# jaswon/osu-dreamer

Hardware: AMD Instinct MI355X
Metric: denoiser train-steps/sec + 50-step sample latents/sec, 1/2/4/8 MI355X (higher is better)
Workload: dtype bf16

## Files before the change

include/osu_dreamer_hip.h:

```cpp
#ifndef OSU_DREAMER_HIP_H
#define OSU_DREAMER_HIP_H

#ifdef __cplusplus
extern "C" {
#endif

enum { OD_F32 = 0, OD_BF16 = 1,
       OD_F32X3 = 2,
       OD_F32X3W = 3,
       OD_F16 = 4 };
enum { OD_EPI_NONE = 0, OD_EPI_SILU = 1 };
enum { OD_ACT_NONE = 0, OD_ACT_SILU = 1 };
enum { OD_ERR_ARG = -1, OD_ERR_ALIGN = -2, OD_ERR_UNSUPPORTED = -3, OD_ERR_COMM = -4 };

int od_version(void);
const char* od_build_source_sha(void);
const char* od_error_string(int code);

int od_gemm_nt(int dtype, const void* A, int lda, const void* W, int ldw, const float* bias, void* C, int ldc,
               int M, int N, int K, int epilogue, int accumulate, void* stream);
int od_gemm_nt_qkrope(int dtype, const void* A, int lda, const void* W, int ldw, const float* bias, void* C, int ldc, int M,
                      int N, int K, const float* wq, const float* wk, const float* table, int L, int H, int hd, float eps,
                      float q_scale, void* stream);
int od_gemm_nt_qkrope_split(int dtype, const void* A, int lda, const void* W, int ldw, const float* bias, void* C, int ldc,
// ... 15 lines not shown
int od_cl_to_frames(int dtype, const float* src, void* dst, int ldd, int B, int C, int L, void* stream);
int od_proj_in(int dtype, const float* xt, const float* W, const float* bias, void* x, int ldx, int B, int E, int L,
               int D, void* stream);
int od_proj_in_bwd(int dtype, const float* xt, const void* dx, int ldx, float* dW, float* db, int B, int E, int L, int D,
                   void* stream);
int od_silu(int dtype, const void* x, void* y, long n, void* stream);
int od_silu_bwd(int dtype, const void* x, const void* dy, void* dx, long n, void* stream);

int od_rmsnorm_film(int dtype, const void* x, int ldx, const float* ssg, const void* cl, int ldcl, int cl_bcast,
                    void* h, int ldh, float* inv_rms, int B, int L, int C, float eps, void* stream);
int od_rmsnorm_film_bwd(int dtype, const void* x, int ldx, const float* inv_rms, const float* ssg, const void* dh,
                        int lddh, void* dres, int lddres, float* dssg, int B, int L, int C, void* stream);
int od_rmsnorm_gate_residual(int dtype, const void* x, int ldx, const void* h, int ldh, const float* ssg, void* xo,
                             int ldxo, float* inv_rms, int B, int L, int C, float eps, void* stream);
int od_rmsnorm_gate_residual_film(int dtype, const void* x, int ldx, const void* h, int ldh, const float* ssg_a, void* xo, int ldxo,
                                  float* inv_a, const float* ssg_b, const void* cl, int ldcl, int cl_bcast, void* h2, int ldh2,
                                  float* inv_b, int B, int L, int C, float eps, void* stream);
int od_rmsnorm_gate_residual_film_dwconv(int dtype, const void* x, int ldx, const void* h, int ldh, const float* ssg_a, void* xo, int ldxo,
                                         float* inv_a, const float* ssg_b, void* h2, int ldh2, float* inv_b, const float* conv_w,
                                         const float* conv_b, void* y, int ldy, int B, int L, int C, int ksize, float eps, void* stream);
int od_rmsnorm_gate_residual_bwd(int dtype, const void* h, int ldh, const float* inv_rms, const float* ssg,
                                 const void* dy, int lddy, void* dh, int lddh, float* dssg, int B, int L, int C,
                                 void* stream);

int od_rope_table(float* table, int L, int hd, void* stream);
int od_qk_norm_rope(int dtype, const void* qkv, int ldqkv, const float* wq, const float* wk, const float* table,
                    void* qk_out, int ldo, int B, int L, int H, int hd, float eps, float q_scale, void* stream);
int od_qk_norm_rope_bwd(int dtype, const void* qkv, int ldqkv, const float* wq, const float* wk, const float* table,
                        const void* dqk, int lddqk, void* dqkv, int lddqkv, float* dwq, float* dwk, int B, int L,
                        int H, int hd, float eps, float q_scale, void* stream);
int od_flash_attn_fwd(int dtype, const void* q, int ldq, const void* k, int ldk, const void* v, int ldv, void* o, int ldo,
                      float* lse, int B, int H, int L, int hd, float scale, int q_prescaled, void* stream);
int od_flash_attn_fwd_varlen(int dtype, const void* q, int ldq, const void* k, int ldk, const void* v, int ldv, void* o, int ldo,
                             float* lse, const int* lens, int B, int H, int L, int hd, float scale, int q_prescaled, void* stream);
int od_flash_attn_bwd(int dtype, const void* q, int ldq, const void* k, int ldk, const void* v, int ldv, const void* o,
                      int ldo, const void* dout, int lddo, const float* lse, float* delta, void* dq, int lddq, void* dk,
                      int lddk, void* dv, int lddv, int B, int H, int L, int hd, float scale, int q_prescaled, void* stream);
int od_attn_aux_create(void** aux_out);
int od_attn_aux_destroy(void* aux);
int od_flash_attn_bwd_aux(int dtype, const void* q, int ldq, const void* k, int ldk, const void* v, int ldv, const void* o,
                          int ldo, const void* dout, int lddo, const float* lse, float* delta, void* dq, int lddq, void* dk,
                          int lddk, void* dv, int lddv, int B, int H, int L, int hd, float scale, int q_prescaled, void* aux, void* stream);
int od_flash_attn_bwd_fused_ws_bytes(int dtype, int B, int H, int L, long* total_out, long* zero_out);
int od_flash_attn_bwd_fused(int dtype, const void* q, int ldq, const void* k, int ldk, const void* v, int ldv, const void* o, int ldo,
                            const void* dout, int lddo, const float* lse, void* dq, int lddq, void* dk, int lddk, void* dv, int lddv,
                            int B, int H, int L, int hd, float scale, int q_prescaled, void* ws, long ws_bytes, void* stream);
// ... 129 lines not shown
```

osu_dreamer_amd/csrc/heads.hip:

```cpp
#include "od_common.h"
#include "od_api_internal.h"

namespace {

constexpr int UW = 32;
constexpr int UOWN = 30;
constexpr int UWPB = 4;
constexpr int MAXU = 64, MAXE = 8;

__device__ __forceinline__ float red32(float v) {
#pragma unroll
    for (int m = 16; m >= 1; m >>= 1) v += __shfl_xor(v, m);
    return v;
}

struct UHeadW {
    const float *w0, *b0, *w1, *b1, *w3, *b3, *w4, *b4;
};

struct UHeadSmem {
    float xts[MAXE][UW + 4];
    float z0s[MAXE][UW + 2];
    float z1s[MAXU][UW + 2];
    float a1s[MAXU][UW + 2];
// ... 17 lines not shown
    }
    __syncthreads();
    for (int idx = t; idx < U * (UW + 2); idx += 256) {
        const int c = idx / (UW + 2), i2 = idx % (UW + 2);
        const int f = l0 - 2 + i2;
        float z = P.b1[c];
        for (int e = 0; e < E; e++) z += P.w1[c * E + e] * S.z0s[e][i2];
        S.z1s[c][i2] = z;
        S.a1s[c][i2] = (f >= 0 && f < Lv) ? od_silu(z) : 0.f;
    }
    __syncthreads();
    for (int idx = t; idx < U * UW; idx += 256) {
        const int c = idx / UW, i = idx % UW;
        S.z3s[c][i] = P.b3[c] + P.w3[c * 3 + 0] * S.a1s[c][i] + P.w3[c * 3 + 1] * S.a1s[c][i + 1] + P.w3[c * 3 + 2] * S.a1s[c][i + 2];
    }
    __syncthreads();
}

__device__ __forceinline__ void uhead_load_w4(UHeadSmem& S, const UHeadW& P, int U) {
    for (int idx = threadIdx.x; idx < U * U; idx += 256) S.w4s[idx / U][idx % U] = P.w4[idx];
    __syncthreads();
}

template <bool VL = false>
__global__ __launch_bounds__(256) void uhead_fwd_kernel(const float* __restrict__ xt, UHeadW P, float* __restrict__ fsum,
                                                        int E, int L, int U, int nwin, int wpb, const OdDetTable* __restrict__ det,
                                                        const int* __restrict__ lens = nullptr) {
    __shared__ UHeadSmem S;
    const int b = blockIdx.y, t = threadIdx.x;
    const int Lb = VL ? od_uniform(lens[b]) : L;
    const int i = t & 31, grp = t >> 5, cpg = U / 8;
    uhead_load_w4(S, P, U);
    float acc[MAXU / 8];
#pragma unroll
    for (int q = 0; q < MAXU / 8; q++) acc[q] = 0.f;
    for (int wi = 0; wi < wpb; wi++) {
        const int win = blockIdx.x * wpb + wi;
        if (win >= nwin) break;
        const int l0 = win * UOWN;
        if (VL && l0 >= Lb) break;
        uhead_window_fwd(S, xt, P, b, l0, E, L, U, Lb);
        const int f = l0 - 1 + i;
        const bool own = (i >= 1 && i < UW - 1 && f < Lb);
#pragma unroll
        for (int q = 0; q < MAXU / 8; q++) {
            if (q < cpg) {
                const int c = grp * cpg + q;
                float z = P.b4[c];
                for (int cc = 0; cc < U; cc++) z += S.w4s[c][cc] * S.z3s[cc][i];
                if (own) acc[q] += od_silu(z);
            }
        }
        __syncthreads();
    }
#pragma unroll
    for (int q = 0; q < MAXU / 8; q++) {
        const float s = red32(acc[q]);
        if (q < cpg && i == 0) od_red_add(det, fsum + (size_t)b * U + grp * cpg + q, s);
    }
}

struct UHeadG {
    float *dw0, *db0, *dw1, *db1, *dw3, *db3, *dw4, *db4;
};

__global__ __launch_bounds__(256) void uhead_bwd_kernel(const float* __restrict__ xt, UHeadW P, const float* __restrict__ dfm,
                                                        UHeadG G, int E, int L, int U, int nwin, const OdDetTable* __restrict__ det) {
    __shared__ UHeadSmem S;
    __shared__ float sdw3[MAXU][3], sdb3[MAXU], sdb4[MAXU], sdw1[MAXU][MAXE], sdb1[MAXU], sdw0[MAXE][3], sdb0[MAXE];
    const int b = blockIdx.y, t = threadIdx.x;
    const int i = t & 31, grp = t >> 5, cpg = U / 8;
    for (int idx = t; idx < MAXU; idx += 256) {
        sdb3[idx] = 0.f; sdb4[idx] = 0.f; sdb1[idx] = 0.f;
        for (int j = 0; j < 3; j++) sdw3[idx][j] = 0.f;
        for (int e = 0; e < MAXE; e++) sdw1[idx][e] = 0.f;
    }
    if (t < MAXE) { sdb0[t] = 0.f; for (int j = 0; j < 3; j++) sdw0[t][j] = 0.f; }
    uhead_load_w4(S, P, U);
    float adw4[16];
#pragma unroll
    for (int q = 0; q < 16; q++) adw4[q] = 0.f;
    const float invL = 1.0f / (float)L;

    for (int wi = 0; wi < UWPB; wi++) {
        const int win = blockIdx.x * UWPB + wi;
        if (win >= nwin) break;
        const int l0 = win * UOWN;
        uhead_window_fwd(S, xt, P, b, l0, E, L, U, L);
        const int f = l0 - 1 + i;
        const bool inr = (f >= 0 && f < L);
        const bool own = (i >= 1 && i < UW - 1 && f < L);
#pragma unroll
        for (int q = 0; q < MAXU / 8; q++) {
            if (q < cpg) {
                const int c = grp * cpg + q;
                float z = P.b4[c];
                for (int cc = 0; cc < U; cc++) z += S.w4s[c][cc] * S.z3s[cc][i];
                const float g = inr ? dfm[(size_t)b * U + c] * invL * od_silu_grad(z) : 0.f;
                S.g4s[c][i] = g;
                const float s = red32(own ? g : 0.f);
                if (i == 0) atomicAdd(&sdb4[c], s);
            }
        }
        __syncthreads();
        {
            const int iend = (L - (l0 - 1)) < (UW - 1) ? (L - (l0 - 1)) : (UW - 1);
#pragma unroll
            for (int q = 0; q < 16; q++) {
                const int o = t + 256 * q;
                if (o < U * U) {
                    const int c = o / U, cc = o % U;
                    float s = 0.f;
                    for (int ii = 1; ii < iend; ii++) s += S.g4s[c][ii] * S.z3s[cc][ii];
                    adw4[q] += s;
                }
            }
        }
        __syncthreads();
        float dz3v[MAXU / 8];
#pragma unroll
        for (int q = 0; q < MAXU / 8; q++) {
            dz3v[q] = 0.f;
            if (q < cpg) {
                const int cc = grp * cpg + q;
                float s = 0.f;
                for (int c = 0; c < U; c++) s += S.w4s[c][cc] * S.g4s[c][i];
                dz3v[q] = s;
            }
        }
        __syncthreads();
#pragma unroll
        for (int q = 0; q < MAXU / 8; q++)
            if (q < cpg) S.z3s[grp * cpg + q][i] = dz3v[q];
        __syncthreads();
#pragma unroll
        for (int q = 0; q < MAXU / 8; q++) {
            if (q < cpg) {
                const int c = grp * cpg + q;
                const float g = own ? S.z3s[c][i] : 0.f;
                float s = red32(g);
                if (i == 0) atomicAdd(&sdb3[c], s);
                for (int j = 0; j < 3; j++) {
                    s = red32(g * S.a1s[c][i + j]);
                    if (i == 0) atomicAdd(&sdw3[c][j], s);
                }
                float dz1 = 0.f;
                if (own) {
                    float da1 = 0.f;
                    for (int j = 0; j < 3; j++) da1 += P.w3[c * 3 + j] * S.z3s[c][i - j + 1];
                    dz1 = da1 * od_silu_grad(S.z1s[c][i + 1]);
                }
                S.g4s[c][i] = dz1;
                s = red32(dz1);
                if (i == 0) atomicAdd(&sdb1[c], s);
                for (int e = 0; e < E; e++) {
                    s = red32(dz1 * S.z0s[e][i + 1]);
                    if (i == 0) atomicAdd(&sdw1[c][e], s);
                }
            }
        }
        __syncthreads();
        {
            const bool ev = grp < E;
            const int e = ev ? grp : 0;
            float dz0 = 0.f;
            if (ev)
                for (int c = 0; c < U; c++) dz0 += P.w1[c * E + e] * S.g4s[c][i];
            float s = red32(dz0);
            if (ev && i == 0) atomicAdd(&sdb0[e], s);
            for (int j = 0; j < 3; j++) {
                s = red32(dz0 * S.xts[e][i + 1 + j]);
                if (ev && i == 0) atomicAdd(&sdw0[e][j], s);
            }
        }
        __syncthreads();
    }
#pragma unroll
    for (int q = 0; q < 16; q++) {
        const int o = t + 256 * q;
        if (o < U * U) od_red_add(det, G.dw4 + o, adw4[q]);
    }
    __syncthreads();
    for (int c = t; c < U; c += 256) {
        od_red_add(det, G.db4 + c, sdb4[c]);
        od_red_add(det, G.db3 + c, sdb3[c]);
        od_red_add(det, G.db1 + c, sdb1[c]);
        for (int j = 0; j < 3; j++) od_red_add(det, G.dw3 + c * 3 + j, sdw3[c][j]);
        for (int e = 0; e < E; e++) od_red_add(det, G.dw1 + c * E + e, sdw1[c][e]);
    }
    if (t < E) {
        od_red_add(det, G.db0 + t, sdb0[t]);
        for (int j = 0; j < 3; j++) od_red_add(det, G.dw0 + t * 3 + j, sdw0[t][j]);
    }
}

template <bool VL = false>
__global__ void uhead_tail_kernel(const float* __restrict__ fsum, const float* __restrict__ mod, const float* __restrict__ w,
                                  const float* __restrict__ bo, float* __restrict__ u, int B, int U, int L, float u_scale,
                                  const int* __restrict__ lens = nullptr) {
    const int b = blockIdx.x, lane = threadIdx.x;
    const float Lf = (float)(VL ? od_uniform(lens[b]) : L);
    float s = 0.f;
    for (int c = lane; c < U; c += 64) {
        const float f = fsum[(size_t)b * U + c] / Lf;
        s += w[c] * (f * (1.f + mod[(size_t)b * 2 * U + c]) + mod[(size_t)b * 2 * U + U + c]);
    }
    s = od_wave_sum(s);
    if (lane == 0) {
        const float y = s + bo[0];
        const float sp = y > 20.f ? y : log1pf(__expf(y));
        u[b] = u_scale * sp;
    }
}
__global__ void uhead_tail_bwd_kernel(const float* __restrict__ fsum, const float* __restrict__ mod, const float* __restrict__ w,
                                      const float* __restrict__ bo, const float* __restrict__ du, float* __restrict__ dfm,
                                      float* __restrict__ dmod, float* __restrict__ dw, float* __restrict__ dbo,
// ... 158 lines not shown
extern "C" int od_uhead_fwd_varlen(const float* xt, const float* w0, const float* b0, const float* w1, const float* b1, const float* w3,
                                   const float* b3, const float* w4, const float* b4, float* fsum, const int* lens, int B, int E, int L,
                                   int U, void* stream) {
    if (U > MAXU || U % 8 || E > MAXE) return OD_ERR_UNSUPPORTED;
    if (!lens) return OD_ERR_ARG;
    const int nwin = (L + UOWN - 1) / UOWN;
    UHeadW P{w0, b0, w1, b1, w3, b3, w4, b4};
    int wpb = (int)((long)nwin * B / 512);
    wpb = wpb < 1 ? 1 : (wpb > UWPB ? UWPB : wpb);
    OD_LAUNCH(uhead_fwd_kernel<true>, dim3((nwin + wpb - 1) / wpb, B), dim3(256), 0, (hipStream_t)stream, xt, P, fsum, E, L, U, nwin, wpb,
              od_det_active(), lens);
    OD_CHECK_LAUNCH();
    return 0;
}

extern "C" int od_uhead_bwd(const float* xt, const float* w0, const float* b0, const float* w1, const float* b1, const float* w3,
                            const float* b3, const float* w4, const float* b4, const float* dfm, float* dw0, float* db0,
                            float* dw1, float* db1, float* dw3, float* db3, float* dw4, float* db4, int B, int E, int L, int U,
                            void* stream) {
    if (U > MAXU || U % 8 || E > MAXE) return OD_ERR_UNSUPPORTED;
    const int nwin = (L + UOWN - 1) / UOWN;
    UHeadW P{w0, b0, w1, b1, w3, b3, w4, b4};
    UHeadG G{dw0, db0, dw1, db1, dw3, db3, dw4, db4};
    OD_LAUNCH(uhead_bwd_kernel, dim3((nwin + UWPB - 1) / UWPB, B), dim3(256), 0, (hipStream_t)stream, xt, P, dfm, G, E, L, U, nwin, od_det_active());
    OD_CHECK_LAUNCH();
    return 0;
}

extern "C" int od_uhead_tail(const float* fsum, const float* mod, const float* w_out, const float* b_out, float* u, int B, int U,
                             int L, float u_scale, void* stream) {
    OD_LAUNCH(uhead_tail_kernel<>, dim3(B), dim3(64), 0, (hipStream_t)stream, fsum, mod, w_out, b_out, u, B, U, L, u_scale);
    OD_CHECK_LAUNCH();
    return 0;
}

extern "C" int od_uhead_tail_varlen(const float* fsum, const float* mod, const float* w_out, const float* b_out, float* u, const int* lens,
                                    int B, int U, int L, float u_scale, void* stream) {
    if (!lens) return OD_ERR_ARG;
    OD_LAUNCH(uhead_tail_kernel<true>, dim3(B), dim3(64), 0, (hipStream_t)stream, fsum, mod, w_out, b_out, u, B, U, L, u_scale, lens);
    OD_CHECK_LAUNCH();
    return 0;
}

extern "C" int od_uhead_tail_bwd(const float* fsum, const float* mod, const float* w_out, const float* b_out, const float* du,
                                 float* dfm, float* dmod, float* dw_out, float* db_out, int B, int U, int L, float u_scale,
                                 void* stream) {
    OD_LAUNCH(uhead_tail_bwd_kernel, dim3(B), dim3(64), 0, (hipStream_t)stream, fsum, mod, w_out, b_out, du, dfm, dmod, dw_out,
// ... 60 lines not shown
```

osu_dreamer_amd/csrc/rowops.hip:

```cpp
#include "od_common.h"
#include "od_api_internal.h"

namespace {

#ifndef OD_QK_BPW
#define OD_QK_BPW 8
#endif
constexpr int ROWS_PER_WAVE_BWD = 16;

template <class T, int NCH>
__device__ __forceinline__ void load_row(const T* row, int C, int lane, float (&v)[NCH][8]) {
#pragma unroll
    for (int i = 0; i < NCH; i++) {
        const int c = (lane + 64 * i) * 8;
        if (c < C) od_ld8(row + c, v[i]);
        else {
#pragma unroll
            for (int e = 0; e < 8; e++) v[i][e] = 0.f;
        }
    }
}
template <int NCH>
__device__ __forceinline__ float row_sumsq(const float (&v)[NCH][8]) {
    float s = 0.f;
// ... 312 lines not shown
#pragma unroll
        for (int i = 0; i < NCH; i++) {
            const int c = (lane + 64 * i) * 8;
            if (c >= C) continue;
            float o[8];
#pragma unroll
            for (int e = 0; e < 8; e++) o[e] = inv * (gv[i][e] - hv[i][e] * dot);
            od_st8(dh + m * lddh + c, o);
        }
    }
    for (int w = 0; w < 4; w++) {
        if (wave == w) {
#pragma unroll
            for (int i = 0; i < NCH; i++)
#pragma unroll
                for (int e = 0; e < 8; e++) {
                    const int idx = (lane + 64 * i) * 8 + e;
                    if (w == 0) red[idx] = dg[i][e]; else red[idx] += dg[i][e];
                }
        }
        __syncthreads();
    }
    for (int c = threadIdx.x; c < C; c += 256) od_red_add(det, dssg + (size_t)b * 3 * C + 2 * C + c, red[c]);
}

template <class T, int NCH>
__global__ __launch_bounds__(256) void swiglu_rmsnorm_kernel(const T* __restrict__ vg, int ldvg, T* __restrict__ hh, int ldhh,
                                                             float* __restrict__ inv_rms, long M, int Hf, int Hp, float eps) {
    const int lane = threadIdx.x & 63;
    const long m = (long)blockIdx.x * 4 + (threadIdx.x >> 6);
    if (m >= M) return;
    float v[NCH][8], g[NCH][8];
    load_row<T, NCH>(vg + m * ldvg, Hp, lane, v);
    load_row<T, NCH>(vg + m * ldvg + Hp, Hp, lane, g);
#pragma unroll
    for (int i = 0; i < NCH; i++)
#pragma unroll
        for (int e = 0; e < 8; e++) v[i][e] *= od_silu(g[i][e]);
    const float inv = rsqrtf(row_sumsq<NCH>(v) / (float)Hf + eps);
    if (lane == 0 && inv_rms) inv_rms[m] = inv;
#pragma unroll
    for (int i = 0; i < NCH; i++) {
        const int c = (lane + 64 * i) * 8;
        if (c >= Hp) continue;
        float o[8];
#pragma unroll
// ... 516 lines not shown
    const bool small = (long)B * ((L + 31) / 32) < OD_FD_SMALL_RUNS;
    const int run = small ? 8 : 32;
    dim3 grid((unsigned)((L + 4 * run - 1) / (4 * run)), (unsigned)B);
#define FD_GO2(T_, KS_, RUN_) OD_LAUNCH((rmsnorm_gate_res_film_dwconv_kernel<T_, KS_, RUN_>), grid, dim3(256), 0, (hipStream_t)stream, (const T_*)x, ldx, \
                   (const T_*)h, ldh, ssg_a, (T_*)xo, ldxo, inv_a, ssg_b, (T_*)h2, ldh2, inv_b, conv_w, conv_b, (T_*)y, ldy, B, L, C, eps)
#define FD_GO1(T_, KS_) do { if (small) FD_GO2(T_, KS_, 8); else FD_GO2(T_, KS_, 32); } while (0)
#define FD_GO(KS_) do { if (dtype == OD_BF16) FD_GO1(bf16_t, KS_); else if (dtype == OD_F32) FD_GO1(float, KS_); else return OD_ERR_UNSUPPORTED; } while (0)
    if (ksize == 5) FD_GO(5); else if (ksize == 3) FD_GO(3); else if (ksize == 7) FD_GO(7); else FD_GO(9);
#undef FD_GO
#undef FD_GO1
#undef FD_GO2
    OD_CHECK_LAUNCH();
    return 0;
}

extern "C" int od_rmsnorm_gate_residual_bwd(int dtype, const void* h, int ldh, const float* inv_rms, const float* ssg,
                                            const void* dy, int lddy, void* dh, int lddh, float* dssg, int B, int L, int C,
                                            void* stream) {
    if (C % 8 || ldh % 8 || lddy % 8 || lddh % 8) return OD_ERR_ALIGN;
    dim3 grid((L + 4 * ROWS_PER_WAVE_BWD - 1) / (4 * ROWS_PER_WAVE_BWD), B);
    DISPATCH_T_NCH(dtype, nch_for(C),
        OD_LAUNCH((rmsnorm_gate_res_bwd_kernel<T_, N_>), grid, dim3(256), 0, (hipStream_t)stream, (const T_*)h, ldh, inv_rms, ssg,
                  (const T_*)dy, lddy, (T_*)dh, lddh, dssg, B, L, C, od_det_active()));
    OD_CHECK_LAUNCH();
    return 0;
}

extern "C" int od_swiglu_rmsnorm(int dtype, const void* vg, int ldvg, void* hh, int ldhh, float* inv_rms, int M, int Hf, int Hp,
                                 float eps, void* stream) {
    if (Hp % 8 || ldvg % 8 || ldhh % 8 || Hf > Hp) return OD_ERR_ALIGN;
    dim3 grid((unsigned)((M + 3) / 4));
    DISPATCH_T_NCH(dtype, nch_for(Hp),
        OD_LAUNCH((swiglu_rmsnorm_kernel<T_, N_>), grid, dim3(256), 0, (hipStream_t)stream, (const T_*)vg, ldvg, (T_*)hh, ldhh, inv_rms,
                  (long)M, Hf, Hp, eps));
    OD_CHECK_LAUNCH();
    return 0;
}

extern "C" int od_swiglu_rmsnorm_bwd(int dtype, const void* vg, int ldvg, const float* inv_rms, const void* dhh, int lddhh,
                                     void* dvg, int lddvg, int M, int Hf, int Hp, void* stream) {
    if (Hp % 8 || ldvg % 8 || lddhh % 8 || lddvg % 8 || Hf > Hp) return OD_ERR_ALIGN;
    dim3 grid((unsigned)((M + 3) / 4));
    DISPATCH_T_NCH(dtype, nch_for(Hp),
        OD_LAUNCH((swiglu_rmsnorm_bwd_kernel<T_, N_>), grid, dim3(256), 0, (hipStream_t)stream, (const T_*)vg, ldvg, inv_rms,
                  (const T_*)dhh, lddhh, (T_*)dvg, lddvg, (long)M, Hf, Hp));
    OD_CHECK_LAUNCH();
// ... 110 lines not shown
```

osu_dreamer_amd/engine.py:

```python
from __future__ import annotations


import math
import os
from typing import Dict, List, Optional

import torch

from . import det, ops
from ._lib import OD_ACT_NONE, OD_ACT_SILU

OD_FUSE_FILM_DWCONV_DEFAULT = "0"

FP32_EPS = float(torch.finfo(torch.float32).eps)


def _ceil(x: int, m: int) -> int:
    return (x + m - 1) // m * m


class Workspace:

    def __init__(self, device):
        self.device = device
# ... 336 lines not shown
    def _uhead_w(self, grads=False):
        f = self.G if grads else self.P
        return [f(f"u_head.{j}.{s}") for j in (0, 1, 3, 4) for s in ("weight", "bias")]

    def backward(self, xt: torch.Tensor, style: torch.Tensor, du: torch.Tensor, dv: torch.Tensor, reducer=None):
        assert self.train
        B, L, M, D, dh, Hf, Hp, A = self.B, self.L, self.M, self.D, self.dh, self.Hf, self.Hp, self.A
        f32 = torch.float32
        dctx = det.context(self.model.arena.data.device)
        if dctx is not None:
            dctx.register(self.model.arena.ensure_grad())
        tab = self.ws.t["rope"]
        cg, a = self.ws.t["cg"], self.ws.t["a"]
        dx = self.buf("d.x", (M, D))
        dbr = self.buf("d.branch", (M, D))
        dtmp = self.buf("d.tmp", (M, D))
        dhh = self.buf("d.hh", (M, Hp))
        dvg = self.buf("d.vg", (M, 2 * Hp))
        dy = self.buf("d.y", (M, dh))
        dqkv = self.buf("d.qkv", (M, 3 * dh))
        da = self.buf("d.a", (self.Ma, A))
        delta = self.buf("d.delta", (B, self.H, L), f32)
        dcg = self.buf("d.cg", (B, self.Cg), f32)
        dssg1, dssg2 = self.buf("d.ssg1", (B, 3 * D), f32), self.buf("d.ssg2", (B, 3 * D), f32)

        ops.final_norm_proj_out_bwd(self._x_last, self.ws.t["invf"], self.P("proj_out.weight"), dv, dx,
                                    self.G("proj_out.weight"), self.G("proj_out.bias"), B, L)
        dfm, dmod = self.buf("d.fm", (B, self.U), f32), self.buf("d.mod", (B, 2 * self.U), f32)
        ops.uhead_tail_bwd(self.ws.t["fsum"], self.ws.t["umod"], self.P("u_out.weight"), self.P("u_out.bias"), du,
                           dfm, dmod, self.G("u_out.weight"), self.G("u_out.bias"), L, self.model.u_scale)
        ops.uhead_bwd(xt, self._uhead_w(), dfm, self._uhead_w(grads=True), self.U)
        ops.linear_small_bwd(cg, self.P("u_mod.weight"), None, dmod, self.buf("d.lin_pre_umod", (B, 2 * self.U), f32),
                             self.G("u_mod.weight"), self.G("u_mod.bias"), dcg, False, OD_ACT_NONE)
        self._det_flush_segment("tail")
        if reducer is not None:
            reducer.segment_done("tail")

        for i in reversed(range(self.depth)):
            p = f"net.layers.{i}."
            t = self.ws.t
            ssg1, ssg2 = t[f"ssg1.{i}"], t[f"ssg2.{i}"]
            dssg1.zero_()
            dssg2.zero_()
            ops.rmsnorm_gate_residual_bwd(t[f"fo.{i}"], t[f"inv5.{i}"], ssg2, dx, dbr, dssg2, B, L)
            ops.gemm_tn(dbr, t[f"hh.{i}"], self.G(p + "ffn.proj_o.weight"), n_cols=D, k_cols=Hf,
                        dbias=self.G(p + "ffn.proj_o.bias"))
            ops.gemm_nt(dbr, self.W(p + "ffn.proj_o", T=True), None, dhh)
            if self._drop_active():
                ops.scale_channels(dhh, self._drop_mask(i), B, L)
            ops.swiglu_rmsnorm_bwd(t[f"vg.{i}"], t[f"inv4.{i}"], dhh, dvg, Hf, Hp)
            gw, gb = self.G(p + "ffn.proj_vg.1.weight"), self.G(p + "ffn.proj_vg.1.bias")
            hdw = t[f"hdw.{i}"] if self.radius > 0 else t[f"h2.{i}"]
            ops.gemm_tn(dvg, hdw, gw, n_cols=2 * Hp, k_cols=D, dbias=gb, n_block=Hp, n_valid=Hf)
            if self.radius > 0:
                self.plain_gemm(dvg, self.W(p + "ffn.proj_vg.1", T=True), None, dtmp)
                ops.dwconv_bwd(t[f"h2.{i}"], self.P(p + "ffn.proj_vg.0.weight"), dtmp, dbr,
                               self.G(p + "ffn.proj_vg.0.weight"), self.G(p + "ffn.proj_vg.0.bias"), B, L, self.ksize)
            else:
                self.plain_gemm(dvg, self.W(p + "ffn.proj_vg.1", T=True), None, dbr)
            ops.rmsnorm_film_bwd(t[f"x_mid.{i}"], t[f"inv3.{i}"], ssg2, dbr, dx, dssg2, B, L)
            ops.rmsnorm_gate_residual_bwd(t[f"ao.{i}"], t[f"inv2.{i}"], ssg1, dx, dbr, dssg1, B, L)
            ops.gemm_tn(dbr, t[f"y.{i}"], self.G(p + "attn.out_proj.weight"), dbias=self.G(p + "attn.out_proj.bias"))
            ops.gemm_nt(dbr, self.W(p + "attn.out_proj", T=True), None, dy)
            self.attn_bwd_launch(i, dy, delta, dqkv)
            ops.gemm_tn(dqkv, t[f"h1.{i}"], self.G(p + "attn.qkv_proj.weight"), dbias=self.G(p + "attn.qkv_proj.bias"))
            self.plain_gemm(dqkv, self.W(p + "attn.qkv_proj", T=True), None, dtmp)
            ops.gemm_tn(dtmp, a, self.G(p + "proj_cl.weight"), dbias=self.G(p + "proj_cl.bias"))
            ops.gemm_nt(dtmp, self.W(p + "proj_cl", T=True), None, da, accumulate=(i != self.depth - 1))
            ops.rmsnorm_film_bwd(t[f"x_in.{i}"], t[f"inv1.{i}"], ssg1, dtmp, dx, dssg1, B, L)
            lp = self.buf("d.lin_pre_ssg", (B, 3 * D), f32)
            self._det_flush(dssg1, dssg2)
            ops.linear_small_bwd(cg, self.P(p + "ssg2.weight"), None, dssg2, lp, self.G(p + "ssg2.weight"),
                                 self.G(p + "ssg2.bias"), dcg, True, OD_ACT_NONE)
            ops.linear_small_bwd(cg, self.P(p + "ssg1.weight"), None, dssg1, lp, self.G(p + "ssg1.weight"),
                                 self.G(p + "ssg1.bias"), dcg, True, OD_ACT_NONE)
            self._det_flush_segment(f"layer{i}")
            if reducer is not None:
                reducer.segment_done(f"layer{i}")

        ops.proj_in_bwd(xt, dx, self.G("proj_in.weight"), self.G("proj_in.bias"))
        da_pre = self.buf("d.a_pre", (self.Ma, A))
        ops.silu_bwd(self.ws.t["a_pre"], da, da_pre)
        ops.gemm_tn(da_pre, self.ws.t["a_t"], self.G("proj_audio.0.weight"), dbias=self.G("proj_audio.0.bias"))
        self._det_flush(dcg)
        ops.linear_small_bwd(style, self.P("proj_style.0.weight"), self.ws.t["cg_pre"], dcg,
                             self.buf("d.lin_pre_style", (B, self.Cg), f32), self.G("proj_style.0.weight"),
                             self.G("proj_style.0.bias"), None, False, OD_ACT_SILU)
        self._det_flush_segment("head")
        if reducer is not None:
            reducer.segment_done("head")
        if self.fused_attn_bwd() and self._attn_ws is not None and not self._attn_ws.checked:
            self._attn_ws.checked = True
# ... 22 lines not shown
```

osu_dreamer_amd/ops.py:

```python
from __future__ import annotations

import os
from typing import Optional

import torch

from . import _lib
from ._lib import OD_ACT_NONE, OD_ACT_SILU, OD_BF16, OD_EPI_NONE, OD_EPI_SILU, OD_F32, OD_F32X3, OD_F32X3W


def dt_code(dtype: torch.dtype) -> int:
    if dtype == torch.float32:
        return OD_F32
    if dtype == torch.bfloat16:
        return OD_BF16
    if dtype == torch.float16:
        return _lib.OD_F16
    raise TypeError(f"unsupported compute dtype {dtype}")


class SplitWeight:

    def __init__(self, storage: torch.Tensor):
        self.t = storage
# ... 168 lines not shown

def rmsnorm_gate_residual_film(x, h, ssg_a, xo, inv_a, ssg_b, cl, cl_bcast, h2, inv_b, B, L, eps=1e-6):
    _f32(ssg_a, ssg_b, inv_a, inv_b)
    _lib.lib().od_rmsnorm_gate_residual_film(dt_code(x.dtype), _p(x), _ld(x), _p(h), _ld(h), _p(ssg_a), _p(xo), _ld(xo),
                                             _p(inv_a), _p(ssg_b), _p(cl), _ld(cl) if cl is not None else 0, int(cl_bcast),
                                             _p(h2), _ld(h2), _p(inv_b), B, L, x.shape[1], eps, _stream(x))


def rmsnorm_gate_residual_film_dwconv(x, h, ssg_a, xo, inv_a, ssg_b, h2, inv_b, conv_w, conv_b, y, B, L, ksize, eps=1e-6):
    _f32(ssg_a, ssg_b, inv_a, inv_b, conv_w, conv_b)
    assert xo.data_ptr() != x.data_ptr() and xo.data_ptr() != h.data_ptr()
    _lib.lib().od_rmsnorm_gate_residual_film_dwconv(dt_code(x.dtype), _p(x), _ld(x), _p(h), _ld(h), _p(ssg_a), _p(xo), _ld(xo), _p(inv_a),
                                                    _p(ssg_b), _p(h2), _ld(h2) if h2 is not None else 0, _p(inv_b), _p(conv_w), _p(conv_b),
                                                    _p(y), _ld(y), B, L, x.shape[1], ksize, eps, _stream(x))


def rmsnorm_gate_residual_bwd(h, inv_rms, ssg, dy, dh, dssg, B, L):
    C = h.shape[1]
    _f32(ssg, inv_rms, dssg)
    _lib.lib().od_rmsnorm_gate_residual_bwd(dt_code(h.dtype), _p(h), _ld(h), _p(inv_rms), _p(ssg), _p(dy), _ld(dy),
                                            _p(dh), _ld(dh), _p(dssg), B, L, C, _stream(h))


def rope_table(table, L, hd):
    _f32(table)
    _lib.lib().od_rope_table(_p(table), L, hd, _stream(table))


def qk_norm_rope(qkv, wq, wk, table, qk_out, B, L, H, hd, eps, q_scale=1.0):
    _f32(wq, wk, table)
    _lib.lib().od_qk_norm_rope(dt_code(qkv.dtype), _p(qkv), _ld(qkv), _p(wq), _p(wk), _p(table), _p(qk_out),
                               _ld(qk_out), B, L, H, hd, eps, q_scale, _stream(qkv))


def qk_norm_rope_bwd(qkv, wq, wk, table, dqk, dqkv, dwq, dwk, B, L, H, hd, eps, q_scale=1.0):
    _f32(wq, wk, table, dwq, dwk)
    _lib.lib().od_qk_norm_rope_bwd(dt_code(qkv.dtype), _p(qkv), _ld(qkv), _p(wq), _p(wk), _p(table), _p(dqk), _ld(dqk),
                                   _p(dqkv), _ld(dqkv), _p(dwq), _p(dwk), B, L, H, hd, eps, q_scale, _stream(qkv))


def flash_attn_fwd(q, k, v, o, lse, B, H, L, hd, scale, x3=False, q_prescaled=False):
    _f32(lse)
    assert q.dtype == k.dtype == v.dtype and (o.dtype == q.dtype or (q.dtype == torch.float16 and o.dtype == torch.bfloat16))
    _lib.lib().od_flash_attn_fwd(mm_code(q.dtype, x3), _p(q), _ld(q), _p(k), _ld(k), _p(v), _ld(v), _p(o), _ld(o), _p(lse),
                                 B, H, L, hd, scale, int(q_prescaled), _stream(q))

# ... 369 lines not shown
```

Baseline: 3.240.

## Fuse adjacent rmsnorm backward kernels and move uhead matmuls onto MFMA

Adds a fused kernel that performs the rmsnorm-FiLM backward and the following gate-residual backward in one pass per row. The engine now chains these across layer boundaries and double-buffers the ssg2 gradient, cutting launches and activation round-trips. The uhead forward and backward kernels also gain an MFMA path for the U×U projection and its weight gradient when U is a multiple of 16. The cross-layer chaining makes the buffer handling subtle, and the MFMA path changes the accumulation order.

```diff
diff --git a/include/osu_dreamer_hip.h b/include/osu_dreamer_hip.h
--- a/include/osu_dreamer_hip.h
+++ b/include/osu_dreamer_hip.h
@@ -61,6 +61,9 @@
 int od_rmsnorm_gate_residual_bwd(int dtype, const void* h, int ldh, const float* inv_rms, const float* ssg,
                                  const void* dy, int lddy, void* dh, int lddh, float* dssg, int B, int L, int C,
                                  void* stream);
+int od_rmsnorm_film_gate_residual_bwd(int dtype, const void* x, int ldx, const float* inv_x, const float* ssg_x, const void* g,
+                                      int ldg, void* dres, int lddres, float* dssg_x, const void* h, int ldh, const float* inv_h,
+                                      const float* ssg_h, void* dh, int lddh, float* dssg_h, int B, int L, int C, void* stream);
 
 int od_rope_table(float* table, int L, int hd, void* stream);
 int od_qk_norm_rope(int dtype, const void* qkv, int ldqkv, const float* wq, const float* wk, const float* table,
diff --git a/osu_dreamer_amd/csrc/heads.hip b/osu_dreamer_amd/csrc/heads.hip
--- a/osu_dreamer_amd/csrc/heads.hip
+++ b/osu_dreamer_amd/csrc/heads.hip
@@ -63,6 +63,22 @@
     __syncthreads();
 }
 
+__device__ __forceinline__ void uhead_z4_mfma(const UHeadSmem& S, const float* __restrict__ b4, int U, int mt, int lane, f32x4& z0, f32x4& z1) {
+    const int r16 = lane & 15, kq = lane >> 4;
+#pragma unroll
+    for (int r = 0; r < 4; r++) { z0[r] = b4[16 * mt + 4 * kq + r]; z1[r] = z0[r]; }
+    for (int k = kq; k < U; k += 4) {
+        const float a = S.w4s[16 * mt + r16][k];
+        z0 = __builtin_amdgcn_mfma_f32_16x16x4f32(a, S.z3s[k][r16], z0, 0, 0, 0);
+        z1 = __builtin_amdgcn_mfma_f32_16x16x4f32(a, S.z3s[k][16 + r16], z1, 0, 0, 0);
+    }
+}
+__device__ __forceinline__ float red16(float v) {
+#pragma unroll
+    for (int m = 8; m >= 1; m >>= 1) v += __shfl_xor(v, m);
+    return v;
+}
+
 template <bool VL = false>
 __global__ __launch_bounds__(256) void uhead_fwd_kernel(const float* __restrict__ xt, UHeadW P, float* __restrict__ fsum,
                                                         int E, int L, int U, int nwin, int wpb, const OdDetTable* __restrict__ det,
@@ -72,6 +88,37 @@
     const int Lb = VL ? od_uniform(lens[b]) : L;
     const int i = t & 31, grp = t >> 5, cpg = U / 8;
     uhead_load_w4(S, P, U);
+    if (U % 16 == 0) {
+        const int wave = od_uniform(t >> 6), lane = t & 63, r16 = lane & 15, kq = lane >> 4;
+        const bool wact = wave < U / 16;
+        f32x4 a0 = (f32x4)(0.f), a1 = (f32x4)(0.f);
+        for (int wi = 0; wi < wpb; wi++) {
+            const int win = blockIdx.x * wpb + wi;
+            if (win >= nwin) break;
+            const int l0 = win * UOWN;
+            if (VL && l0 >= Lb) break;
+            uhead_window_fwd(S, xt, P, b, l0, E, L, U, Lb);
+            if (wact) {
+                f32x4 z0, z1;
+                uhead_z4_mfma(S, P.b4, U, wave, lane, z0, z1);
+                const bool own0 = r16 >= 1 && l0 - 1 + r16 < Lb, own1 = r16 < 15 && l0 + 15 + r16 < Lb;
+#pragma unroll
+                for (int r = 0; r < 4; r++) {
+                    if (own0) a0[r] += od_silu(z0[r]);
+                    if (own1) a1[r] += od_silu(z1[r]);
+                }
+            }
+            __syncthreads();
+        }
+        if (wact) {
+#pragma unroll
+            for (int r = 0; r < 4; r++) {
+                const float s = red16(a0[r] + a1[r]);
+                if (r16 == 0) od_red_add(det, fsum + (size_t)b * U + 16 * wave + 4 * kq + r, s);
+            }
+        }
+        return;
+    }
     float acc[MAXU / 8];
 #pragma unroll
     for (int q = 0; q < MAXU / 8; q++) acc[q] = 0.f;
@@ -105,8 +152,9 @@
     float *dw0, *db0, *dw1, *db1, *dw3, *db3, *dw4, *db4;
 };
 
-__global__ __launch_bounds__(256) void uhead_bwd_kernel(const float* __restrict__ xt, UHeadW P, const float* __restrict__ dfm,
-                                                        UHeadG G, int E, int L, int U, int nwin, const OdDetTable* __restrict__ det) {
+template <bool MF>
+__device__ __forceinline__ void uhead_bwd_block(const float* __restrict__ xt, const UHeadW& P, const float* __restrict__ dfm,
+                                                const UHeadG& G, int E, int L, int U, int nwin, const OdDetTable* __restrict__ det) {
     __shared__ UHeadSmem S;
     __shared__ float sdw3[MAXU][3], sdb3[MAXU], sdb4[MAXU], sdw1[MAXU][MAXE], sdb1[MAXU], sdw0[MAXE][3], sdb0[MAXE];
     const int b = blockIdx.y, t = threadIdx.x;
@@ -122,6 +170,12 @@
 #pragma unroll
     for (int q = 0; q < 16; q++) adw4[q] = 0.f;
     const float invL = 1.0f / (float)L;
+    constexpr bool mf = MF;
+    const int wave = od_uniform(t >> 6), lane = t & 63, r16 = lane & 15, kq = lane >> 4, mtiles = U / 16;
+    const bool wact = wave < mtiles;
+    f32x4 adw[4];
+#pragma unroll
+    for (int nt = 0; nt < 4; nt++) adw[nt] = (f32x4)(0.f);
 
     for (int wi = 0; wi < UWPB; wi++) {
         const int win = blockIdx.x * UWPB + wi;
@@ -131,49 +185,99 @@
         const int f = l0 - 1 + i;
         const bool inr = (f >= 0 && f < L);
         const bool own = (i >= 1 && i < UW - 1 && f < L);
-#pragma unroll
-        for (int q = 0; q < MAXU / 8; q++) {
-            if (q < cpg) {
-                const int c = grp * cpg + q;
-                float z = P.b4[c];
-                for (int cc = 0; cc < U; cc++) z += S.w4s[c][cc] * S.z3s[cc][i];
-                const float g = inr ? dfm[(size_t)b * U + c] * invL * od_silu_grad(z) : 0.f;
-                S.g4s[c][i] = g;
-                const float s = red32(own ? g : 0.f);
-                if (i == 0) atomicAdd(&sdb4[c], s);
-            }
+        if constexpr (mf) {
+            if (wact) {
+                f32x4 z0, z1;
+                uhead_z4_mfma(S, P.b4, U, wave, lane, z0, z1);
+                const int f0 = l0 - 1 + r16, f1 = f0 + 16;
+                const bool inr0 = f0 >= 0 && f0 < L, inr1 = f1 < L;
+                const bool own0 = r16 >= 1 && f0 < L, own1 = r16 < 15 && f1 < L;
+#pragma unroll
+                for (int r = 0; r < 4; r++) {
+                    const int c = 16 * wave + 4 * kq + r;
+                    const float d = dfm[(size_t)b * U + c] * invL;
+                    const float g0 = inr0 ? d * od_silu_grad(z0[r]) : 0.f, g1 = inr1 ? d * od_silu_grad(z1[r]) : 0.f;
+                    S.g4s[c][r16] = g0;
+                    S.g4s[c][16 + r16] = g1;
+                    const float s = red16((own0 ? g0 : 0.f) + (own1 ? g1 : 0.f));
+                    if (r16 == 0) sdb4[c] += s;
+                }
+            }
+            __syncthreads();
+            f32x4 d0 = (f32x4)(0.f), d1 = (f32x4)(0.f);
+            if (wact) {
+                f32x4 sw[4];
+#pragma unroll
+                for (int nt = 0; nt < 4; nt++) sw[nt] = (f32x4)(0.f);
+#pragma unroll
+                for (int k = kq; k < UW; k += 4) {
+                    const float av = (k == 0 || k == UW - 1) ? 0.f : S.g4s[16 * wave + r16][k];
+#pragma unroll
+                    for (int nt = 0; nt < 4; nt++)
+                        if (nt < mtiles) sw[nt] = __builtin_amdgcn_mfma_f32_16x16x4f32(av, S.z3s[16 * nt + r16][k], sw[nt], 0, 0, 0);
+                }
+#pragma unroll
+                for (int nt = 0; nt < 4; nt++) adw[nt] += sw[nt];
+                for (int k = kq; k < U; k += 4) {
+                    const float av = S.w4s[k][16 * wave + r16];
+                    d0 = __builtin_amdgcn_mfma_f32_16x16x4f32(av, S.g4s[k][r16], d0, 0, 0, 0);
+                    d1 = __builtin_amdgcn_mfma_f32_16x16x4f32(av, S.g4s[k][16 + r16], d1, 0, 0, 0);
+                }
+            }
+            __syncthreads();
+            if (wact) {
+#pragma unroll
+                for (int r = 0; r < 4; r++) {
+                    S.z3s[16 * wave + 4 * kq + r][r16] = d0[r];
+                    S.z3s[16 * wave + 4 * kq + r][16 + r16] = d1[r];
+                }
+            }
+            __syncthreads();
+        } else {
+#pragma unroll
+            for (int q = 0; q < MAXU / 8; q++) {
+                if (q < cpg) {
+                    const int c = grp * cpg + q;
+                    float z = P.b4[c];
+                    for (int cc = 0; cc < U; cc++) z += S.w4s[c][cc] * S.z3s[cc][i];
+                    const float g = inr ? dfm[(size_t)b * U + c] * invL * od_silu_grad(z) : 0.f;
+                    S.g4s[c][i] = g;
+                    const float s = red32(own ? g : 0.f);
+                    if (i == 0) atomicAdd(&sdb4[c], s);
+                }
+            }
+            __syncthreads();
+            {
+                const int iend = (L - (l0 - 1)) < (UW - 1) ? (L - (l0 - 1)) : (UW - 1);
+#pragma unroll
+                for (int q = 0; q < 16; q++) {
+                    const int o = t + 256 * q;
+                    if (o < U * U) {
+                        const int c = o / U, cc = o % U;
+                        float s = 0.f;
+                        for (int ii = 1; ii < iend; ii++) s += S.g4s[c][ii] * S.z3s[cc][ii];
+                        adw4[q] += s;
+                    }
+                }
+            }
+            __syncthreads();
+            float dz3v[MAXU / 8];
+#pragma unroll
+            for (int q = 0; q < MAXU / 8; q++) {
+                dz3v[q] = 0.f;
+                if (q < cpg) {
+                    const int cc = grp * cpg + q;
+                    float s = 0.f;
+                    for (int c = 0; c < U; c++) s += S.w4s[c][cc] * S.g4s[c][i];
+                    dz3v[q] = s;
+                }
+            }
+            __syncthreads();
+#pragma unroll
+            for (int q = 0; q < MAXU / 8; q++)
+                if (q < cpg) S.z3s[grp * cpg + q][i] = dz3v[q];
+            __syncthreads();
         }
-        __syncthreads();
-        {
-            const int iend = (L - (l0 - 1)) < (UW - 1) ? (L - (l0 - 1)) : (UW - 1);
-#pragma unroll
-            for (int q = 0; q < 16; q++) {
-                const int o = t + 256 * q;
-                if (o < U * U) {
-                    const int c = o / U, cc = o % U;
-                    float s = 0.f;
-                    for (int ii = 1; ii < iend; ii++) s += S.g4s[c][ii] * S.z3s[cc][ii];
-                    adw4[q] += s;
-                }
-            }
-        }
-        __syncthreads();
-        float dz3v[MAXU / 8];
-#pragma unroll
-        for (int q = 0; q < MAXU / 8; q++) {
-            dz3v[q] = 0.f;
-            if (q < cpg) {
-                const int cc = grp * cpg + q;
-                float s = 0.f;
-                for (int c = 0; c < U; c++) s += S.w4s[c][cc] * S.g4s[c][i];
-                dz3v[q] = s;
-            }
-        }
-        __syncthreads();
-#pragma unroll
-        for (int q = 0; q < MAXU / 8; q++)
-            if (q < cpg) S.z3s[grp * cpg + q][i] = dz3v[q];
-        __syncthreads();
 #pragma unroll
         for (int q = 0; q < MAXU / 8; q++) {
             if (q < cpg) {
@@ -219,7 +323,14 @@
 #pragma unroll
     for (int q = 0; q < 16; q++) {
         const int o = t + 256 * q;
-        if (o < U * U) od_red_add(det, G.dw4 + o, adw4[q]);
+        if (!mf && o < U * U) od_red_add(det, G.dw4 + o, adw4[q]);
+    }
+    if (mf && wact) {
+#pragma unroll
+        for (int nt = 0; nt < 4; nt++)
+#pragma unroll
+            for (int r = 0; r < 4; r++)
+                if (nt < mtiles) od_red_add(det, G.dw4 + (size_t)(16 * wave + 4 * kq + r) * U + 16 * nt + r16, adw[nt][r]);
     }
     __syncthreads();
     for (int c = t; c < U; c += 256) {
@@ -233,6 +344,15 @@
         od_red_add(det, G.db0 + t, sdb0[t]);
         for (int j = 0; j < 3; j++) od_red_add(det, G.dw0 + t * 3 + j, sdw0[t][j]);
     }
+}
+
+__global__ __launch_bounds__(256) void uhead_bwd_kernel(const float* __restrict__ xt, UHeadW P, const float* __restrict__ dfm,
+                                                        UHeadG G, int E, int L, int U, int nwin, const OdDetTable* __restrict__ det) {
+    uhead_bwd_block<false>(xt, P, dfm, G, E, L, U, nwin, det);
+}
+__global__ __launch_bounds__(256) void uhead_bwd_mfma_kernel(const float* __restrict__ xt, UHeadW P, const float* __restrict__ dfm,
+                                                             UHeadG G, int E, int L, int U, int nwin, const OdDetTable* __restrict__ det) {
+    uhead_bwd_block<true>(xt, P, dfm, G, E, L, U, nwin, det);
 }
 
 template <bool VL = false>
@@ -437,7 +557,10 @@
     const int nwin = (L + UOWN - 1) / UOWN;
     UHeadW P{w0, b0, w1, b1, w3, b3, w4, b4};
     UHeadG G{dw0, db0, dw1, db1, dw3, db3, dw4, db4};
-    OD_LAUNCH(uhead_bwd_kernel, dim3((nwin + UWPB - 1) / UWPB, B), dim3(256), 0, (hipStream_t)stream, xt, P, dfm, G, E, L, U, nwin, od_det_active());
+    if (U % 16 == 0)
+        OD_LAUNCH(uhead_bwd_mfma_kernel, dim3((nwin + UWPB - 1) / UWPB, B), dim3(256), 0, (hipStream_t)stream, xt, P, dfm, G, E, L, U, nwin, od_det_active());
+    else
+        OD_LAUNCH(uhead_bwd_kernel, dim3((nwin + UWPB - 1) / UWPB, B), dim3(256), 0, (hipStream_t)stream, xt, P, dfm, G, E, L, U, nwin, od_det_active());
     OD_CHECK_LAUNCH();
     return 0;
 }
diff --git a/osu_dreamer_amd/csrc/rowops.hip b/osu_dreamer_amd/csrc/rowops.hip
--- a/osu_dreamer_amd/csrc/rowops.hip
+++ b/osu_dreamer_amd/csrc/rowops.hip
@@ -358,6 +358,115 @@
         __syncthreads();
     }
     for (int c = threadIdx.x; c < C; c += 256) od_red_add(det, dssg + (size_t)b * 3 * C + 2 * C + c, red[c]);
+}
+
+template <class T> struct FgRaw;
+template <> struct FgRaw<bf16_t> { u32x4 v; };
+template <> struct FgRaw<float> { f32x4 a, b; };
+__device__ __forceinline__ void fg_load(FgRaw<bf16_t>& r, const bf16_t* p) { r.v = *(const u32x4*)p; }
+__device__ __forceinline__ void fg_load(FgRaw<float>& r, const float* p) { r.a = *(const f32x4*)p; r.b = *(const f32x4*)(p + 4); }
+__device__ __forceinline__ void fg_zero(FgRaw<bf16_t>& r) { r.v = (u32x4)(0u); }
+__device__ __forceinline__ void fg_zero(FgRaw<float>& r) { r.a = (f32x4)(0.f); r.b = (f32x4)(0.f); }
+__device__ __forceinline__ void fg_unpack(const FgRaw<bf16_t>& r, float (&v)[8]) {
+#pragma unroll
+    for (int i = 0; i < 4; i++) {
+        union { uint32_t u; float f; } lo, hi;
+        lo.u = r.v[i] << 16; hi.u = r.v[i] & 0xffff0000u;
+        v[2 * i] = lo.f; v[2 * i + 1] = hi.f;
+    }
+}
+__device__ __forceinline__ void fg_unpack(const FgRaw<float>& r, float (&v)[8]) {
+#pragma unroll
+    for (int i = 0; i < 4; i++) { v[i] = r.a[i]; v[4 + i] = r.b[i]; }
+}
+template <class T>
+__global__ __launch_bounds__(256) void rmsnorm_film_gate_res_bwd_kernel(const T* __restrict__ x, int ldx, const float* __restrict__ inv_x,
+                                                                        const float* __restrict__ ssg_x, const T* g, int ldg,
+                                                                        T* __restrict__ dres, int lddres, float* __restrict__ dssg_x,
+                                                                        const T* __restrict__ h, int ldh, const float* __restrict__ inv_h,
+                                                                        const float* __restrict__ ssg_h, T* dh, int lddh,
+                                                                        float* __restrict__ dssg_h, int B, int L, int C,
+                                                                        const OdDetTable* __restrict__ det) {
+    __shared__ float red[3][512];
+    const int lane = threadIdx.x & 63, wave = od_uniform(threadIdx.x >> 6);
+    const int b = blockIdx.y;
+    const int l0 = (blockIdx.x * 4 + wave) * ROWS_PER_WAVE_BWD;
+    const int c = lane * 8;
+    const bool act = c < C;
+    const int cl = act ? c : 0;
+    float dsc[8], dsh[8], dg[8], scl[8], gate[8];
+#pragma unroll
+    for (int e = 0; e < 8; e++) { dsc[e] = 0.f; dsh[e] = 0.f; dg[e] = 0.f; scl[e] = 0.f; gate[e] = 0.f; }
+    if (act) {
+        od_ld8(ssg_x + (size_t)b * 3 * C + c, scl);
+        od_ld8(ssg_h + (size_t)b * 3 * C + 2 * C + c, gate);
+    }
+    const int nrow = L - l0 < ROWS_PER_WAVE_BWD ? L - l0 : ROWS_PER_WAVE_BWD;
+    const long m0 = (long)b * L + l0;
+    FgRaw<T> rx, rg, rd, rh;
+    fg_zero(rx); fg_zero(rg); fg_zero(rd); fg_zero(rh);
+    float ninv_x = 0.f, ninv_h = 0.f;
+    if (nrow > 0) {
+        fg_load(rx, x + m0 * ldx + cl); fg_load(rg, g + m0 * ldg + cl); fg_load(rd, dres + m0 * lddres + cl); fg_load(rh, h + m0 * ldh + cl);
+        ninv_x = inv_x[m0]; ninv_h = inv_h[m0];
+    }
+#pragma unroll 1
+    for (int r = 0; r < nrow; r++) {
+        const long m = m0 + r;
+        float xv[8], gv[8], o[8], hv[8];
+        fg_unpack(rx, xv); fg_unpack(rg, gv); fg_unpack(rd, o); fg_unpack(rh, hv);
+        float inv = ninv_x;
+        const float invh = ninv_h;
+        if (r + 1 < nrow) {
+            fg_load(rx, x + (m + 1) * ldx + cl); fg_load(rg, g + (m + 1) * ldg + cl);
+            fg_load(rd, dres + (m + 1) * lddres + cl); fg_load(rh, h + (m + 1) * ldh + cl);
+            ninv_x = inv_x[m + 1]; ninv_h = inv_h[m + 1];
+        }
+        float dot = 0.f;
+#pragma unroll
+        for (int e = 0; e < 8; e++) {
+            const float xh = xv[e] * inv;
+            dsc[e] += gv[e] * xh;
+            dsh[e] += gv[e];
+            gv[e] *= (1.f + scl[e]);
+            dot += gv[e] * xh;
+            xv[e] = xh;
+        }
+        dot = od_wave_sum(act ? dot : 0.f) / (float)C;
+#pragma unroll
+        for (int e = 0; e < 8; e++) o[e] += inv * (gv[e] - xv[e] * dot);
+        if (act) od_st8(dres + m * lddres + c, o);
+        inv = invh; dot = 0.f;
+#pragma unroll
+        for (int e = 0; e < 8; e++) {
+            o[e] = od_round_to<T>(o[e]);
+            const float hh = hv[e] * inv;
+            dg[e] += o[e] * hh;
+            o[e] *= gate[e];
+            dot += o[e] * hh;
+            hv[e] = hh;
+        }
+        dot = od_wave_sum(act ? dot : 0.f) / (float)C;
+#pragma unroll
+        for (int e = 0; e < 8; e++) o[e] = inv * (o[e] - hv[e] * dot);
+        if (act) od_st8(dh + m * lddh + c, o);
+    }
+    for (int w = 0; w < 4; w++) {
+        if (wave == w) {
+#pragma unroll
+            for (int e = 0; e < 8; e++) {
+                const int idx = lane * 8 + e;
+                if (w == 0) { red[0][idx] = dsc[e]; red[1][idx] = dsh[e]; red[2][idx] = dg[e]; }
+                else { red[0][idx] += dsc[e]; red[1][idx] += dsh[e]; red[2][idx] += dg[e]; }
+            }
+        }
+        __syncthreads();
+    }
+    for (int cc = threadIdx.x; cc < C; cc += 256) {
+        od_red_add(det, dssg_x + (size_t)b * 3 * C + cc, red[0][cc]);
+        od_red_add(det, dssg_x + (size_t)b * 3 * C + C + cc, red[1][cc]);
+        od_red_add(det, dssg_h + (size_t)b * 3 * C + 2 * C + cc, red[2][cc]);
+    }
 }
 
 template <class T, int NCH>
@@ -920,6 +1029,23 @@
     DISPATCH_T_NCH(dtype, nch_for(C),
         OD_LAUNCH((rmsnorm_gate_res_bwd_kernel<T_, N_>), grid, dim3(256), 0, (hipStream_t)stream, (const T_*)h, ldh, inv_rms, ssg,
                   (const T_*)dy, lddy, (T_*)dh, lddh, dssg, B, L, C, od_det_active()));
+    OD_CHECK_LAUNCH();
+    return 0;
+}
+
+extern "C" int od_rmsnorm_film_gate_residual_bwd(int dtype, const void* x, int ldx, const float* inv_x, const float* ssg_x, const void* g,
+                                                 int ldg, void* dres, int lddres, float* dssg_x, const void* h, int ldh,
+                                                 const float* inv_h, const float* ssg_h, void* dh, int lddh, float* dssg_h, int B, int L,
+                                                 int C, void* stream) {
+    if (C % 8 || ldx % 8 || ldg % 8 || lddres % 8 || ldh % 8 || lddh % 8) return OD_ERR_ALIGN;
+    if (C > 512) return OD_ERR_UNSUPPORTED;
+    if (dres == g || dres == dh || dres == x || dres == h) return OD_ERR_ARG;
+    dim3 grid((L + 4 * ROWS_PER_WAVE_BWD - 1) / (4 * ROWS_PER_WAVE_BWD), B);
+#define FG_GO(T_) OD_LAUNCH((rmsnorm_film_gate_res_bwd_kernel<T_>), grid, dim3(256), 0, (hipStream_t)stream, (const T_*)x, ldx, inv_x, ssg_x, \
+                            (const T_*)g, ldg, (T_*)dres, lddres, dssg_x, (const T_*)h, ldh, inv_h, ssg_h, (T_*)dh, lddh, dssg_h, B, L, C,    \
+                            od_det_active())
+    if (dtype == OD_BF16) FG_GO(bf16_t); else if (dtype == OD_F32) FG_GO(float); else return OD_ERR_ARG;
+#undef FG_GO
     OD_CHECK_LAUNCH();
     return 0;
 }
diff --git a/osu_dreamer_amd/engine.py b/osu_dreamer_amd/engine.py
--- a/osu_dreamer_amd/engine.py
+++ b/osu_dreamer_amd/engine.py
@@ -382,7 +382,9 @@
         da = self.buf("d.a", (self.Ma, A))
         delta = self.buf("d.delta", (B, self.H, L), f32)
         dcg = self.buf("d.cg", (B, self.Cg), f32)
-        dssg1, dssg2 = self.buf("d.ssg1", (B, 3 * D), f32), self.buf("d.ssg2", (B, 3 * D), f32)
+        fuse_rows = D <= 512
+        dssg1, dssg2_ab = self.buf("d.ssg1", (B, 3 * D), f32), self.buf("d.ssg2", (2, B, 3 * D), f32)
+        dssg2_ab[(self.depth - 1) & 1].zero_()
 
         ops.final_norm_proj_out_bwd(self._x_last, self.ws.t["invf"], self.P("proj_out.weight"), dv, dx,
                                     self.G("proj_out.weight"), self.G("proj_out.bias"), B, L)
@@ -400,9 +402,11 @@
             p = f"net.layers.{i}."
             t = self.ws.t
             ssg1, ssg2 = t[f"ssg1.{i}"], t[f"ssg2.{i}"]
+            dssg2 = dssg2_ab[i & 1]
             dssg1.zero_()
-            dssg2.zero_()
-            ops.rmsnorm_gate_residual_bwd(t[f"fo.{i}"], t[f"inv5.{i}"], ssg2, dx, dbr, dssg2, B, L)
+            dssg2_ab[(i - 1) & 1].zero_()
+            if not (fuse_rows and i != self.depth - 1):
+                ops.rmsnorm_gate_residual_bwd(t[f"fo.{i}"], t[f"inv5.{i}"], ssg2, dx, dbr, dssg2, B, L)
             ops.gemm_tn(dbr, t[f"hh.{i}"], self.G(p + "ffn.proj_o.weight"), n_cols=D, k_cols=Hf,
                         dbias=self.G(p + "ffn.proj_o.bias"))
             ops.gemm_nt(dbr, self.W(p + "ffn.proj_o", T=True), None, dhh)
@@ -418,8 +422,12 @@
                                self.G(p + "ffn.proj_vg.0.weight"), self.G(p + "ffn.proj_vg.0.bias"), B, L, self.ksize)
             else:
                 self.plain_gemm(dvg, self.W(p + "ffn.proj_vg.1", T=True), None, dbr)
-            ops.rmsnorm_film_bwd(t[f"x_mid.{i}"], t[f"inv3.{i}"], ssg2, dbr, dx, dssg2, B, L)
-            ops.rmsnorm_gate_residual_bwd(t[f"ao.{i}"], t[f"inv2.{i}"], ssg1, dx, dbr, dssg1, B, L)
+            if fuse_rows:
+                ops.rmsnorm_film_gate_residual_bwd(t[f"x_mid.{i}"], t[f"inv3.{i}"], ssg2, dbr, dx, dssg2,
+                                                   t[f"ao.{i}"], t[f"inv2.{i}"], ssg1, dbr, dssg1, B, L)
+            else:
+                ops.rmsnorm_film_bwd(t[f"x_mid.{i}"], t[f"inv3.{i}"], ssg2, dbr, dx, dssg2, B, L)
+                ops.rmsnorm_gate_residual_bwd(t[f"ao.{i}"], t[f"inv2.{i}"], ssg1, dx, dbr, dssg1, B, L)
             ops.gemm_tn(dbr, t[f"y.{i}"], self.G(p + "attn.out_proj.weight"), dbias=self.G(p + "attn.out_proj.bias"))
             ops.gemm_nt(dbr, self.W(p + "attn.out_proj", T=True), None, dy)
             self.attn_bwd_launch(i, dy, delta, dqkv)
@@ -427,7 +435,11 @@
             self.plain_gemm(dqkv, self.W(p + "attn.qkv_proj", T=True), None, dtmp)
             ops.gemm_tn(dtmp, a, self.G(p + "proj_cl.weight"), dbias=self.G(p + "proj_cl.bias"))
             ops.gemm_nt(dtmp, self.W(p + "proj_cl", T=True), None, da, accumulate=(i != self.depth - 1))
-            ops.rmsnorm_film_bwd(t[f"x_in.{i}"], t[f"inv1.{i}"], ssg1, dtmp, dx, dssg1, B, L)
+            if fuse_rows and i > 0:
+                ops.rmsnorm_film_gate_residual_bwd(t[f"x_in.{i}"], t[f"inv1.{i}"], ssg1, dtmp, dx, dssg1,
+                                                   t[f"fo.{i - 1}"], t[f"inv5.{i - 1}"], t[f"ssg2.{i - 1}"], dbr, dssg2_ab[(i - 1) & 1], B, L)
+            else:
+                ops.rmsnorm_film_bwd(t[f"x_in.{i}"], t[f"inv1.{i}"], ssg1, dtmp, dx, dssg1, B, L)
             lp = self.buf("d.lin_pre_ssg", (B, 3 * D), f32)
             self._det_flush(dssg1, dssg2)
             ops.linear_small_bwd(cg, self.P(p + "ssg2.weight"), None, dssg2, lp, self.G(p + "ssg2.weight"),
diff --git a/osu_dreamer_amd/ops.py b/osu_dreamer_amd/ops.py
--- a/osu_dreamer_amd/ops.py
+++ b/osu_dreamer_amd/ops.py
@@ -214,6 +214,14 @@
                                             _p(dh), _ld(dh), _p(dssg), B, L, C, _stream(h))
 
 
+def rmsnorm_film_gate_residual_bwd(x, inv_x, ssg_x, g, dres, dssg_x, h, inv_h, ssg_h, dh, dssg_h, B, L):
+    C = x.shape[1]
+    _f32(ssg_x, inv_x, dssg_x, ssg_h, inv_h, dssg_h)
+    _lib.lib().od_rmsnorm_film_gate_residual_bwd(dt_code(x.dtype), _p(x), _ld(x), _p(inv_x), _p(ssg_x), _p(g), _ld(g), _p(dres), _ld(dres),
+                                                 _p(dssg_x), _p(h), _ld(h), _p(inv_h), _p(ssg_h), _p(dh), _ld(dh), _p(dssg_h), B, L, C,
+                                                 _stream(x))
+
+
 def rope_table(table, L, hd):
     _f32(table)
     _lib.lib().od_rope_table(_p(table), L, hd, _stream(table))
```

Measured after the change: 3.257 (median of 6 runs). No clear change (+0.5%).
